# rvaser/rala

Measured on AMD Instinct MI355X. Metric: overlaps/sec (pile build + transitive reduction), higher is better.
Workload: dtype u16/u32 (+f64 compares)

## Files before the change

### rala_amd/csrc/bucket_kernels.hip

```cpp
#include <hip/hip_runtime.h>

#include <algorithm>

#include "device_utils.h"
#include "geom.h"
#include "kernels.h"
#include "scan_pass.h"

namespace rala_hip {

namespace {

constexpr uint32_t kInf = 0xFFFFFFFFu;
constexpr uint32_t kTile = 4096;
constexpr uint32_t kBlockP = 512;
constexpr uint32_t kPer = kTile / kBlockP;
constexpr uint32_t kL1Shift = 12;
constexpr uint32_t kL1Reads = 1u << kL1Shift;
constexpr uint32_t kGroupShift = 7;
constexpr uint32_t kGroupReads = 1u << kGroupShift;
constexpr uint32_t kGroupsPerPart = kL1Reads / kGroupReads;
constexpr uint32_t kKeyBits = 14;
constexpr uint32_t kCoordBits = 25;
constexpr uint32_t kCoordMax = (1u << kCoordBits) - 1u;
static_assert(kKeyBits + 2 * kCoordBits == 64, "a record is 8 bytes");

struct PartGeom {
    uint32_t shift, gpp, n_part;
};
inline PartGeom part_geom(uint32_t n_reads, const BucketTuning& bt) {
    uint32_t shift = kL1Shift;
    while (shift < kKeyBits && ((uint64_t)n_reads + (1u << shift) - 1) >> shift > 256) ++shift;
    if (bt.part_shift >= kL1Shift && bt.part_shift <= kKeyBits) shift = bt.part_shift;
    return PartGeom{shift, 1u << (shift - kGroupShift), (uint32_t)(((uint64_t)n_reads + (1u << shift) - 1) >> shift)};
}

constexpr uint32_t kCountWindow = 150u * 1024u / 4u;
inline uint32_t count_window(const BucketTuning& bt) { return bt.count_window ? bt.count_window : kCountWindow; }

__device__ __forceinline__ uint64_t pack_record(uint32_t b, uint32_t begin, uint32_t end) {
    return (uint64_t)(b & ((1u << kKeyBits) - 1u)) << (2 * kCoordBits) | (uint64_t)(begin < kCoordMax ? begin : kCoordMax) << kCoordBits |
           (uint64_t)(end < kCoordMax ? end : kCoordMax);
}
__device__ __forceinline__ uint32_t rec_key(uint64_t r) { return (uint32_t)(r >> (2 * kCoordBits)); }
__device__ __forceinline__ uint2 rec_events(uint64_t r, uint32_t shrink) {
    const uint32_t begin = (uint32_t)(r >> kCoordBits) & kCoordMax, end = (uint32_t)r & kCoordMax;
    return make_uint2((begin + shrink) << 1, ((end - shrink) << 1) | 1u);
}

__device__ __forceinline__ uint32_t segment_of(uint32_t key, bool active, uint32_t lane, uint32_t& leader) {
    const uint32_t prev = (uint32_t)__shfl_up((int)key, 1, 64);
    const bool prev_active = __shfl_up((int)active, 1, 64) != 0;
    const bool head = active && (lane == 0 || !prev_active || prev != key);
    const uint64_t heads = __ballot(head);
    const uint64_t act = __ballot(active);
    const uint64_t below = heads & ((lane == 63) ? ~0ull : ((2ull << lane) - 1ull));
    leader = below ? 63u - (uint32_t)__clzll((long long)below) : lane;
    const uint64_t after = (lane == 63) ? 0ull : ((heads | ~act) >> (lane + 1));
    const uint32_t len = after ? (uint32_t)__ffsll((unsigned long long)after) : (64u - lane);
    return head ? len : 0u;
}

constexpr uint32_t kBlockC = 1024;
constexpr uint32_t kCountPer = 8;
__global__ __launch_bounds__(kBlockC) void group_count_kernel(OvlSoA o, uint32_t n_reads, uint32_t g_lo, uint32_t n_groups, uint32_t* group_count) {
    extern __shared__ uint32_t s_hist[];
    for (uint32_t g = threadIdx.x; g < n_groups; g += kBlockC) s_hist[g] = 0;
    __syncthreads();
    constexpr uint32_t kC = kCountPer;
    const uint64_t last = o.n - 1;
    for (uint64_t i0 = (uint64_t)blockIdx.x * kBlockC * kC; i0 < o.n; i0 += (uint64_t)gridDim.x * kBlockC * kC) {
        uint32_t a[kC], b[kC];
#pragma unroll
        for (uint32_t u = 0; u < kC; ++u) {
            const uint64_t i = i0 + u * kBlockC + threadIdx.x;
            const uint64_t j = i < o.n ? i : last;
            a[u] = i < o.n ? __builtin_nontemporal_load(o.a_id + j) : kInf;
            b[u] = __builtin_nontemporal_load(o.b_id + j);
        }
#pragma unroll
        for (uint32_t u = 0; u < kC; ++u) {
            const uint32_t g = (b[u] >> kGroupShift) - g_lo;
            if (a[u] < n_reads && b[u] < n_reads && g < n_groups) atomicAdd(&s_hist[g], 1u);
        }
    }
    __syncthreads();
    for (uint32_t g = threadIdx.x; g < n_groups; g += kBlockC) {
        const uint32_t c = s_hist[g];
        if (c) atomicAdd(&group_count[g_lo + g], c);
    }
}

__device__ __forceinline__ void load4_ids(const uint32_t* p, uint64_t i0, uint64_t n, uint32_t (&out)[4]) {
    typedef uint32_t u32x4_t __attribute__((ext_vector_type(4)));
    if (i0 + 4 <= n) {
        const u32x4_t v = __builtin_nontemporal_load((const u32x4_t*)(p + i0));
        out[0] = v.x; out[1] = v.y; out[2] = v.z; out[3] = v.w;
    } else {
#pragma unroll
        for (uint32_t e = 0; e < 4; ++e) out[e] = i0 + e < n ? p[i0 + e] : kInf;
    }
}
constexpr uint32_t kCountVec = 2;
constexpr uint32_t kFlagStage = 512;
template <bool kShard>
__global__ __launch_bounds__(kBlockC) void group_count_dedupe_kernel(OvlSoA o, uint32_t n_reads, uint32_t n_groups, uint32_t* group_count,
                                                                     uint8_t* __restrict__ suspect, uint8_t* __restrict__ valid, uint32_t* list_pos,
                                                                     uint32_t* list_query, uint32_t list_cap, uint32_t* list_count,
                                                                     uint32_t world, uint32_t groups) {
    extern __shared__ uint32_t s_hist[];
    __shared__ uint32_t s_fpos[kFlagStage], s_fq[kFlagStage], s_fcnt, s_fbase;
    for (uint32_t g = threadIdx.x; g < n_groups; g += kBlockC) s_hist[g] = 0;
    if (threadIdx.x == 0) s_fcnt = 0;
    __syncthreads();
    const uint32_t lane = threadIdx.x & 63;
    auto mark = [&](uint32_t query, uint64_t at) {
        suspect[query] = 1;
        const uint32_t slot = atomicAdd(&s_fcnt, 1u);
        if (slot < kFlagStage) { s_fpos[slot] = (uint32_t)at; s_fq[slot] = query; }
    };
    constexpr uint64_t kTrip = (uint64_t)kBlockC * 4 * kCountVec;
    for (uint64_t c0 = (uint64_t)blockIdx.x * kTrip; c0 < o.n; c0 += (uint64_t)gridDim.x * kTrip) {
        uint32_t a[kCountVec][4], b[kCountVec][4];
#pragma unroll
        for (uint32_t u = 0; u < kCountVec; ++u) {
            const uint64_t i0 = c0 + ((uint64_t)u * kBlockC + threadIdx.x) * 4;
            load4_ids(o.a_id, i0, o.n, a[u]);
            load4_ids(o.b_id, i0, o.n, b[u]);
        }
#pragma unroll
        for (uint32_t u = 0; u < kCountVec; ++u) {
            const uint64_t i0 = c0 + ((uint64_t)u * kBlockC + threadIdx.x) * 4;
            uint32_t pa = (uint32_t)__shfl_up((int)a[u][3], 1, 64), pb = (uint32_t)__shfl_up((int)b[u][3], 1, 64);
            if (lane == 0 && i0 > 0 && i0 < o.n) { pa = o.a_id[i0 - 1]; pb = o.b_id[i0 - 1]; }
            bool have_prev = i0 > 0;
            uint32_t word = 0;
#pragma unroll
            for (uint32_t e = 0; e < 4; ++e) {
                const uint32_t x = a[u][e], y = b[u][e];
                const bool in = i0 + e < o.n;
                const bool ok = in && x < n_reads && y < n_reads;
                if (ok) {
                    if constexpr (kShard) {
                        atomicAdd(&s_hist[(x % world) * groups + ((x / world) >> kGroupShift)], 1u);
                        atomicAdd(&s_hist[(y % world) * groups + ((y / world) >> kGroupShift)], 1u);
                    } else {
                        if ((y >> kGroupShift) < n_groups) atomicAdd(&s_hist[y >> kGroupShift], 1u);
                    }
                }
                if (in && have_prev) {
                    const bool pok = pa < n_reads && pb < n_reads;
                    if (ok && pok) {
                        if (pa == x && y <= pb) mark(x, i0 + e);
                    } else {
                        if (x < n_reads) mark(x, i0 + e);
                        if (pa < n_reads) mark(pa, i0 + e - 1);
                    }
                }
                if (ok && x != y) word |= 1u << (8 * e);
                pa = x; pb = y; have_prev = true;
            }
            if (i0 + 4 <= o.n) *(uint32_t*)(valid + i0) = word;
            else for (uint32_t e = 0; e < 4 && i0 + e < o.n; ++e) valid[i0 + e] = (uint8_t)(word >> (8 * e));
        }
        __syncthreads();
        const uint32_t staged = s_fcnt;
        if (staged) {
            if (threadIdx.x == 0) s_fbase = staged > kFlagStage ? atomicOr(list_count, kDedupeListGivenUp) : atomicAdd(list_count, staged);
            __syncthreads();
            if (staged <= kFlagStage) {
                for (uint32_t k = threadIdx.x; k < staged; k += kBlockC) {
                    const uint32_t at = s_fbase + k;
                    if (at < list_cap) { list_pos[at] = s_fpos[k]; list_query[at] = s_fq[k]; }
                }
            }
            __syncthreads();
            if (threadIdx.x == 0) s_fcnt = 0;
            __syncthreads();
        }
    }
    for (uint32_t g = threadIdx.x; g < n_groups; g += kBlockC) {
        const uint32_t c = s_hist[g];
        if (c) atomicAdd(&group_count[g], c);
    }
}

__global__ __launch_bounds__(1024) void layout_kernel(const uint32_t* __restrict__ group_count, uint32_t n_part, uint32_t gpp,
                                                      uint32_t* __restrict__ group_base, uint32_t* __restrict__ group_cursor,
                                                      uint32_t* __restrict__ part_cursor, uint32_t* __restrict__ tile_part,
                                                      uint32_t* __restrict__ tile_lo, uint32_t* __restrict__ tile_hi, uint32_t* n_tiles) {
    __shared__ uint32_t tmp[1024 / 64 + 1];
    const uint32_t n = n_part * gpp;
    uint32_t carry = 0;
    for (uint32_t g0 = 0; g0 < n; g0 += 1024) {
        const uint32_t g = g0 + threadIdx.x;
        const uint32_t c = g < n ? group_count[g] : 0u;
        uint32_t tot;
        const uint32_t ex = block_scan_excl<1024>(c, OpAdd(), 0u, tmp, tot);
        if (g < n) {
            group_base[g] = carry + ex;
            group_cursor[g] = carry + ex;
            if (g % gpp == 0) part_cursor[g / gpp] = carry + ex;
        }
        carry += tot;
    }
    if (threadIdx.x == 0) group_base[n] = carry;
    __syncthreads();
    uint32_t tile_carry = 0;
    for (uint32_t p0 = 0; p0 < n_part; p0 += 1024) {
        const uint32_t p = p0 + threadIdx.x;
        const uint32_t lo = p < n_part ? group_base[p * gpp] : 0u;
        const uint32_t hi = p < n_part ? group_base[(p + 1u) * gpp] : 0u;
        const uint32_t tiles = (hi - lo + kTile - 1) / kTile;
        uint32_t ttot;
        const uint32_t tex = block_scan_excl<1024>(tiles, OpAdd(), 0u, tmp, ttot);
        for (uint32_t k = 0; k < tiles; ++k) {
            tile_part[tile_carry + tex + k] = p;
            tile_lo[tile_carry + tex + k] = lo + k * kTile;
            tile_hi[tile_carry + tex + k] = umin(hi, lo + (k + 1u) * kTile);
        }
        tile_carry += ttot;
    }
    if (threadIdx.x == 0) *n_tiles = tile_carry;
}

struct StageLds {
    uint64_t* stage;
    uint16_t* bin_of;
    uint32_t *hist, *off, *gbase;
    __device__ StageLds(unsigned char* base, uint32_t n_bins) {
        stage = (uint64_t*)base;
        bin_of = (uint16_t*)(stage + kTile);
        hist = (uint32_t*)(bin_of + kTile);
        off = hist + n_bins;
        gbase = off + n_bins;
    }
};
inline size_t stage_lds_bytes(uint32_t n_bins) { return (size_t)kTile * 10 + (size_t)n_bins * 12 + 16; }

__device__ __forceinline__ void stage_and_copy(StageLds& L, uint32_t n_bins, const uint64_t* rec, const uint32_t* bin, const bool* in,
                                               uint32_t* cursor, uint64_t* __restrict__ out, uint32_t* tmp) {
    for (uint32_t p = threadIdx.x; p < n_bins; p += kBlockP) L.hist[p] = 0;
    __syncthreads();
    uint32_t rank[kPer];
#pragma unroll
    for (uint32_t u = 0; u < kPer; ++u) rank[u] = in[u] ? atomicAdd(&L.hist[bin[u]], 1u) : 0u;
    __syncthreads();
    uint32_t carry = 0;
    for (uint32_t p0 = 0; p0 < n_bins; p0 += kBlockP) {
        const uint32_t p = p0 + threadIdx.x;
        const uint32_t c = p < n_bins ? L.hist[p] : 0u;
        uint32_t tot;
        const uint32_t ex = block_scan_excl<(int)kBlockP>(c, OpAdd(), 0u, tmp, tot);
        if (p < n_bins) {
            L.off[p] = carry + ex;
            L.gbase[p] = c ? atomicAdd(&cursor[p], c) : 0u;
        }
        carry += tot;
    }
    __syncthreads();
    const uint32_t total = carry;
#pragma unroll
    for (uint32_t u = 0; u < kPer; ++u) {
        if (in[u]) {
            const uint32_t at = L.off[bin[u]] + rank[u];
            L.stage[at] = rec[u];
            L.bin_of[at] = (uint16_t)bin[u];
        }
    }
    __syncthreads();
    for (uint32_t j = threadIdx.x; j < total; j += kBlockP) {
        const uint32_t p = L.bin_of[j];
        out[L.gbase[p] + (j - L.off[p])] = L.stage[j];
    }
}

__global__ __launch_bounds__(kBlockP) void l1_scatter_kernel(OvlSoA o, uint32_t n_reads, uint32_t n_part, uint32_t shift, uint32_t* part_cursor,
                                                             uint64_t* __restrict__ rec1, uint32_t* acount) {
    extern __shared__ __align__(16) unsigned char s_raw[];
    __shared__ uint32_t tmp[kBlockP / 64 + 1];
    StageLds L(s_raw, n_part);
    uint64_t rec[kPer];
    uint32_t bin[kPer];
    bool in[kPer];
    const uint32_t lane = threadIdx.x & 63;
    const uint64_t last = o.n - 1;
#pragma unroll
    for (uint32_t u = 0; u < kPer; ++u) {
        const uint64_t i = (uint64_t)blockIdx.x * kTile + u * kBlockP + threadIdx.x;
        const uint64_t j = i < o.n ? i : last;
        const uint32_t a = o.a_id[j], b = o.b_id[j];
        in[u] = i < o.n && a < n_reads && b < n_reads;
        rec[u] = pack_record(b, o.b_begin[j], o.b_end[j]);
        bin[u] = in[u] ? b >> shift : 0u;
        uint32_t leader;
        const uint32_t seg = segment_of(a, in[u], lane, leader);
        if (seg) atomicAdd(&acount[a], seg);
    }
    stage_and_copy(L, n_part, rec, bin, in, part_cursor, rec1, tmp);
}

__device__ __forceinline__ uint32_t bound_record_read(uint64_t r) { return (uint32_t)(r >> (2 * kBoundRecordCoordBits)); }

__global__ __launch_bounds__(kBlockC) void group_count_records_kernel(const uint64_t* __restrict__ records, uint64_t n, uint32_t n_reads,
                                                                      uint32_t g_lo, uint32_t n_groups, uint32_t* group_count) {
    extern __shared__ uint32_t s_hist[];
    for (uint32_t g = threadIdx.x; g < n_groups; g += kBlockC) s_hist[g] = 0;
    __syncthreads();
    constexpr uint32_t kC = kCountPer;
    for (uint64_t i0 = (uint64_t)blockIdx.x * kBlockC * kC; i0 < n; i0 += (uint64_t)gridDim.x * kBlockC * kC) {
        uint32_t key[kC];
#pragma unroll
        for (uint32_t u = 0; u < kC; ++u) {
            const uint64_t i = i0 + u * kBlockC + threadIdx.x;
            key[u] = i < n ? bound_record_read(__builtin_nontemporal_load(records + i)) : kInf;
        }
#pragma unroll
        for (uint32_t u = 0; u < kC; ++u) {
            const uint32_t g = (key[u] >> kGroupShift) - g_lo;
            if (key[u] < n_reads && g < n_groups) atomicAdd(&s_hist[g], 1u);
        }
    }
    __syncthreads();
    for (uint32_t g = threadIdx.x; g < n_groups; g += kBlockC) {
        const uint32_t c = s_hist[g];
        if (c) atomicAdd(&group_count[g_lo + g], c);
    }
}

__global__ __launch_bounds__(kBlockP) void l1_scatter_records_kernel(const uint64_t* __restrict__ records, uint64_t n, uint32_t n_reads,
                                                                     uint32_t n_part, uint32_t shift, uint32_t* part_cursor, uint64_t* __restrict__ rec1) {
    extern __shared__ __align__(16) unsigned char s_raw[];
    __shared__ uint32_t tmp[kBlockP / 64 + 1];
    StageLds L(s_raw, n_part);
    uint64_t rec[kPer];
    uint32_t bin[kPer];
    bool in[kPer];
    constexpr uint32_t kMask = (1u << kBoundRecordCoordBits) - 1u;
#pragma unroll
    for (uint32_t u = 0; u < kPer; ++u) {
        const uint64_t i = (uint64_t)blockIdx.x * kTile + u * kBlockP + threadIdx.x;
        const uint64_t r = i < n ? __builtin_nontemporal_load(records + i) : ~0ull;
        const uint32_t key = bound_record_read(r);
        in[u] = i < n && key < n_reads;
        rec[u] = pack_record(key, (uint32_t)(r >> kBoundRecordCoordBits) & kMask, (uint32_t)r & kMask);
        bin[u] = in[u] ? key >> shift : 0u;
    }
    stage_and_copy(L, n_part, rec, bin, in, part_cursor, rec1, tmp);
}

constexpr uint32_t kTileOtherBase = 0x80000000u;
__global__ __launch_bounds__(kBlockP) void l2_scatter_kernel(const uint64_t* __restrict__ rec1, const uint64_t* __restrict__ rec1b,
                                                             const uint32_t* __restrict__ tile_part,
                                                             const uint32_t* __restrict__ tile_lo, const uint32_t* __restrict__ tile_hi,
                                                             const uint32_t* __restrict__ n_tiles, uint32_t* group_cursor,
                                                             uint64_t* __restrict__ rec2, uint32_t gpp) {
    extern __shared__ __align__(16) unsigned char s_raw[];
    __shared__ uint32_t tmp[kBlockP / 64 + 1];
    if (blockIdx.x >= *n_tiles) return;
    StageLds L(s_raw, gpp);
    const uint32_t part_mask = gpp * kGroupReads - 1u;
    const uint32_t part_word = tile_part[blockIdx.x], lo = tile_lo[blockIdx.x], hi = tile_hi[blockIdx.x];
    const uint32_t part = part_word & ~kTileOtherBase;
    const uint64_t* __restrict__ src = (part_word & kTileOtherBase) ? rec1b : rec1;
    uint64_t rec[kPer];
    uint32_t bin[kPer];
    bool in[kPer];
#pragma unroll
    for (uint32_t u = 0; u < kPer; ++u) {
        const uint32_t j = lo + u * kBlockP + threadIdx.x;
        in[u] = j < hi;
        rec[u] = in[u] ? src[j] : 0ull;
        bin[u] = (rec_key(rec[u]) & part_mask) >> kGroupShift;
    }
    stage_and_copy(L, gpp, rec, bin, in, group_cursor + part * gpp, rec2, tmp);
}

__global__ __launch_bounds__(kGroupReads) void group_query_sum_kernel(const uint32_t* __restrict__ acount, uint32_t n_reads,
                                                                      uint32_t* __restrict__ qsum) {
    __shared__ uint32_t tmp[kGroupReads / 64 + 1];
    const uint32_t r = blockIdx.x * kGroupReads + threadIdx.x;
    const uint32_t v = block_reduce<(int)kGroupReads>(r < n_reads ? acount[r] : 0u, OpAdd(), 0u, tmp);
    if (threadIdx.x == 0) qsum[blockIdx.x] = v;
}

__global__ __launch_bounds__(1024) void group_event_base_kernel(const uint32_t* __restrict__ qsum, const uint32_t* __restrict__ group_base,
                                                                uint32_t n_groups, uint32_t* __restrict__ pair_base) {
    __shared__ uint32_t tmp[1024 / 64 + 1];
    uint32_t carry = 0;
    for (uint32_t g0 = 0; g0 < n_groups; g0 += 1024) {
        const uint32_t g = g0 + threadIdx.x;
        const uint32_t c = g < n_groups ? qsum[g] + (group_base[g + 1] - group_base[g]) : 0u;
        uint32_t tot;
        const uint32_t ex = block_scan_excl<1024>(c, OpAdd(), 0u, tmp, tot);
        if (g < n_groups) pair_base[g] = carry + ex;
        carry += tot;
    }
    if (threadIdx.x == 0) pair_base[n_groups] = carry;
}

__global__ __launch_bounds__(kBlockP) void final_kernel(const uint64_t* __restrict__ rec2, const uint32_t* __restrict__ group_base,
                                                        const uint32_t* __restrict__ pair_base, uint32_t n_reads,
                                                        const uint32_t* __restrict__ acount, uint32_t* __restrict__ ev_off,
                                                        uint32_t* __restrict__ ev, uint32_t shrink, uint32_t ev_shift) {
    extern __shared__ __align__(16) unsigned char s_raw[];
    __shared__ uint32_t tmp[kBlockP / 64 + 1];
    __shared__ uint32_t s_cursor[kGroupReads];
    __shared__ uint32_t s_cnt[kGroupReads];
    static_assert(kGroupReads <= kBlockP, "one thread per read of the group");
    StageLds L(s_raw, kGroupReads);
    const uint32_t g = blockIdx.x;
    if (threadIdx.x < kGroupReads) s_cnt[threadIdx.x] = 0;
    __syncthreads();
    const uint32_t lo = group_base[g], hi = group_base[g + 1];
    uint64_t first[kPer];
#pragma unroll
    for (uint32_t u = 0; u < kPer; ++u) {
        const uint32_t j = lo + u * kBlockP + threadIdx.x;
        first[u] = j < hi ? rec2[j] : 0ull;
        if (j < hi) atomicAdd(&s_cnt[rec_key(first[u]) & (kGroupReads - 1u)], 1u);
    }
    for (uint32_t j = lo + kTile + threadIdx.x; j < hi; j += kBlockP) atomicAdd(&s_cnt[rec_key(rec2[j]) & (kGroupReads - 1u)], 1u);
    __syncthreads();
    {
        const uint32_t r = g * kGroupReads + threadIdx.x;
        const bool mine = threadIdx.x < kGroupReads && r < n_reads;
        const uint32_t q = mine && acount ? acount[r] : 0u;
        const uint32_t pairs = mine ? q + s_cnt[threadIdx.x] : 0u;
        uint32_t tot;
        const uint32_t before = pair_base[g] + block_scan_excl<(int)kBlockP>(pairs, OpAdd(), 0u, tmp, tot);
        if (mine) {
            ev_off[r] = before << (1u - ev_shift);
            s_cursor[threadIdx.x] = before + q;
            if (r == n_reads - 1u) ev_off[n_reads] = (before + pairs) << (1u - ev_shift);
        }
    }
    __syncthreads();
    for (uint32_t j0 = lo; j0 < hi; j0 += kTile) {
        uint64_t pair[kPer];
        uint32_t bin[kPer];
        bool in[kPer];
#pragma unroll
        for (uint32_t u = 0; u < kPer; ++u) {
            const uint32_t j = j0 + u * kBlockP + threadIdx.x;
            in[u] = j < hi;
            const uint64_t rec = j0 == lo ? first[u] : in[u] ? rec2[j] : 0ull;
            const uint2 e = rec_events(rec, shrink);
            pair[u] = (uint64_t)e.x | (uint64_t)e.y << 32;
            bin[u] = rec_key(rec) & (kGroupReads - 1u);
        }
        stage_and_copy(L, kGroupReads, pair, bin, in, s_cursor, (uint64_t*)ev, tmp);
        __syncthreads();
    }
}

template <uint32_t kQ>
__global__ __launch_bounds__(256) void query_side_kernel(OvlSoA o, uint32_t n_reads, const uint32_t* __restrict__ ev_off,
                                                         uint32_t* written, uint32_t* __restrict__ ev, uint32_t ev_shift) {
    const uint32_t lane = threadIdx.x & 63;
    uint32_t a[kQ], b[kQ], begin[kQ], end[kQ];
#pragma unroll
    for (uint32_t u = 0; u < kQ; ++u) {
        const uint64_t i = ((uint64_t)blockIdx.x * kQ + u) * 256 + threadIdx.x;
        a[u] = kInf; b[u] = kInf; begin[u] = 0; end[u] = 0;
        if (i < o.n) { a[u] = o.a_id[i]; b[u] = o.b_id[i]; begin[u] = __builtin_nontemporal_load(o.a_begin + i); end[u] = __builtin_nontemporal_load(o.a_end + i); }
    }
    uint32_t base[kQ], leader[kQ];
    bool ok[kQ];
#pragma unroll
    for (uint32_t u = 0; u < kQ; ++u) {
        ok[u] = a[u] < n_reads && b[u] < n_reads;
        const uint32_t seg = segment_of(a[u], ok[u], lane, leader[u]);
        base[u] = 0;
        if (seg) base[u] = ev_off[a[u]] + atomicAdd(&written[a[u]], (2u >> ev_shift) * seg);
    }
#pragma unroll
    for (uint32_t u = 0; u < kQ; ++u) {
        const uint32_t at = (uint32_t)__shfl((int)base[u], (int)leader[u], 64);
        if (ok[u]) *(uint2*)(ev + ((size_t)at << ev_shift) + 2u * (lane - leader[u])) = make_uint2((begin[u] + 15u) << 1, ((end[u] - 15u) << 1) | 1u);
    }
}


__global__ __launch_bounds__(kBlockC) void shard_count_kernel(OvlSoA o, uint32_t n_reads, uint32_t world, uint32_t groups,
                                                              uint32_t n_bins, uint32_t* group_count) {
    extern __shared__ uint32_t s_hist[];
    for (uint32_t g = threadIdx.x; g < n_bins; g += kBlockC) s_hist[g] = 0;
    __syncthreads();
    constexpr uint32_t kC = kCountPer;
    const uint64_t last = o.n - 1;
    for (uint64_t i0 = (uint64_t)blockIdx.x * kBlockC * kC; i0 < o.n; i0 += (uint64_t)gridDim.x * kBlockC * kC) {
        uint32_t a[kC], b[kC];
#pragma unroll
        for (uint32_t u = 0; u < kC; ++u) {
            const uint64_t i = i0 + u * kBlockC + threadIdx.x;
            const uint64_t j = i < o.n ? i : last;
            a[u] = i < o.n ? __builtin_nontemporal_load(o.a_id + j) : kInf;
            b[u] = __builtin_nontemporal_load(o.b_id + j);
        }
#pragma unroll
        for (uint32_t u = 0; u < kC; ++u) {
            if (a[u] < n_reads && b[u] < n_reads) {
                atomicAdd(&s_hist[(a[u] % world) * groups + ((a[u] / world) >> kGroupShift)], 1u);
                atomicAdd(&s_hist[(b[u] % world) * groups + ((b[u] / world) >> kGroupShift)], 1u);
            }
        }
    }
    __syncthreads();
    for (uint32_t g = threadIdx.x; g < n_bins; g += kBlockC) {
        const uint32_t c = s_hist[g];
        if (c) atomicAdd(&group_count[g], c);
    }
}

__global__ __launch_bounds__(1024) void shard_send_layout_kernel(const uint32_t* __restrict__ group_count, ShardGeometry g,
                                                                 uint64_t* __restrict__ send, uint32_t* __restrict__ part_cursor,
                                                                 uint32_t* __restrict__ send_words) {
    __shared__ uint32_t tmp[1024 / 64 + 1];
    uint32_t block_start = 0;
    for (uint32_t p = 0; p < g.world; ++p) {
        uint32_t* header = (uint32_t*)(send + block_start);
        uint32_t carry = block_start + g.header;
        for (uint32_t g0 = 0; g0 < g.groups; g0 += 1024) {
            const uint32_t k = g0 + threadIdx.x;
            const uint32_t c = k < g.groups ? group_count[p * g.groups + k] : 0u;
            uint32_t tot;
            const uint32_t ex = block_scan_excl<1024>(c, OpAdd(), 0u, tmp, tot);
            if (k < g.groups) {
                header[k] = c;
                if (k % kGroupsPerPart == 0) part_cursor[p * g.n_part + k / kGroupsPerPart] = carry + ex;
            }
            carry += tot;
        }
        if (threadIdx.x == 0) send_words[p] = carry - block_start;
        block_start = carry;
    }
}

__global__ __launch_bounds__(kBlockP) void shard_l1_scatter_kernel(OvlSoA o, uint32_t n_reads, uint32_t world, uint32_t n_part,
                                                                   uint32_t* part_cursor, uint64_t* __restrict__ send) {
    extern __shared__ __align__(16) unsigned char s_raw[];
    __shared__ uint32_t tmp[kBlockP / 64 + 1];
    const uint32_t n_bins = world * n_part;
    StageLds L(s_raw, n_bins);
    uint64_t rec[kPer];
    uint32_t bin[kPer];
    bool in[kPer];
    const uint64_t last = o.n - 1;
    static_assert(kPer % 2 == 0, "two records per overlap");
#pragma unroll
    for (uint32_t u = 0; u < kPer / 2; ++u) {
        const uint64_t i = (uint64_t)blockIdx.x * (kTile / 2) + u * kBlockP + threadIdx.x;
        const uint64_t j = i < o.n ? i : last;
        const uint32_t a = o.a_id[j], b = o.b_id[j];
        const bool ok = i < o.n && a < n_reads && b < n_reads;
        const uint32_t la = a / world, lb = b / world;
        in[2 * u] = in[2 * u + 1] = ok;
        rec[2 * u] = pack_record(la, __builtin_nontemporal_load(o.a_begin + j), __builtin_nontemporal_load(o.a_end + j));
        rec[2 * u + 1] = pack_record(lb, __builtin_nontemporal_load(o.b_begin + j), __builtin_nontemporal_load(o.b_end + j));
        bin[2 * u] = ok ? (a - la * world) * n_part + (la >> kL1Shift) : 0u;
        bin[2 * u + 1] = ok ? (b - lb * world) * n_part + (lb >> kL1Shift) : 0u;
    }
    stage_and_copy(L, n_bins, rec, bin, in, part_cursor, send, tmp);
}

__global__ __launch_bounds__(1024) void shard_owner_layout_kernel(const uint64_t* __restrict__ base, const uint64_t* __restrict__ base_self,
                                                                  ShardBlocks blocks, ShardGeometry g,
                                                                  uint32_t* __restrict__ group_base, uint32_t* __restrict__ group_cursor,
                                                                  uint32_t* __restrict__ pair_pref, uint32_t* __restrict__ tile_part,
                                                                  uint32_t* __restrict__ tile_lo, uint32_t* __restrict__ tile_hi,
                                                                  uint32_t* n_tiles) {
    __shared__ uint32_t tmp[1024 / 64 + 1];
    auto header_of = [&](uint32_t p) { return (const uint32_t*)((p == blocks.self ? base_self : base) + blocks.off[p]); };
    uint32_t carry = 0;
    for (uint32_t g0 = 0; g0 < g.groups; g0 += 1024) {
        const uint32_t k = g0 + threadIdx.x;
        uint32_t c = 0;
        if (k < g.groups) {
            for (uint32_t p = 0; p < g.world; ++p) c += header_of(p)[k];
        }
        uint32_t tot;
        const uint32_t ex = block_scan_excl<1024>(c, OpAdd(), 0u, tmp, tot);
        if (k < g.groups) { group_base[k] = carry + ex; group_cursor[k] = carry + ex; }
        carry += tot;
    }
    if (threadIdx.x == 0) group_base[g.groups] = carry;
    const uint32_t n_pairs = g.world * g.n_part;
    uint32_t pcarry = 0;
    for (uint32_t j0 = 0; j0 < n_pairs; j0 += 1024) {
        const uint32_t j = j0 + threadIdx.x;
        uint32_t len = 0;
        if (j < n_pairs) {
            const uint32_t* header = header_of(j / g.n_part) + (j % g.n_part) * kGroupsPerPart;
            for (uint32_t k = 0; k < kGroupsPerPart; ++k) len += header[k];
        }
        uint32_t tot;
        const uint32_t ex = block_scan_excl<1024>(len, OpAdd(), 0u, tmp, tot);
        if (j < n_pairs) pair_pref[j] = pcarry + ex;
        pcarry += tot;
    }
    if (threadIdx.x == 0) pair_pref[n_pairs] = pcarry;
    __syncthreads();
    uint32_t tile_carry = 0;
    for (uint32_t j0 = 0; j0 < n_pairs; j0 += 1024) {
        const uint32_t j = j0 + threadIdx.x;
        uint32_t lo = 0, len = 0, tiles = 0;
        if (j < n_pairs) {
            const uint32_t p = j / g.n_part;
            len = pair_pref[j + 1] - pair_pref[j];
            lo = blocks.off[p] + g.header + (pair_pref[j] - pair_pref[p * g.n_part]);
            tiles = (len + kTile - 1) / kTile;
        }
        uint32_t ttot;
        const uint32_t tex = block_scan_excl<1024>(tiles, OpAdd(), 0u, tmp, ttot);
        for (uint32_t k = 0; k < tiles; ++k) {
            tile_part[tile_carry + tex + k] = (j % g.n_part) | (j / g.n_part == blocks.self ? kTileOtherBase : 0u);
            tile_lo[tile_carry + tex + k] = lo + k * kTile;
            tile_hi[tile_carry + tex + k] = umin(lo + len, lo + (k + 1u) * kTile);
        }
        tile_carry += ttot;
    }
    if (threadIdx.x == 0) *n_tiles = tile_carry;
}

}

uint32_t partition_count(uint32_t n_reads, const BucketTuning& bt) { return part_geom(n_reads, bt).n_part; }
uint32_t partition_group_slots(uint32_t n_reads, const BucketTuning& bt) { const PartGeom G = part_geom(n_reads, bt); return G.n_part * G.gpp + 2; }
size_t partition_records_needed(uint32_t, uint64_t n_overlaps) { return (size_t)n_overlaps + 64; }
size_t partition_tile_slots(uint32_t n_reads, uint64_t n_overlaps, const BucketTuning& bt) { return (size_t)(n_overlaps / kTile) + partition_count(n_reads, bt) + 4; }
bool partition_path_fits(uint32_t n_reads, uint32_t max_read_len, uint64_t n_overlaps, const BucketTuning& bt) {
    if (n_reads == 0 || n_overlaps == 0) return false;
    const PartGeom G = part_geom(n_reads, bt);
    const uint64_t n_part = G.n_part;
    return max_read_len < kCoordMax - 32u && n_part * G.gpp <= 8ull * kCountWindow &&
           stage_lds_bytes((uint32_t)n_part) <= 60u * 1024u && 2ull * n_overlaps < 0xFFFFFFF0ull && n_overlaps / n_part >= 512;
}

namespace {
struct PartitionBuffers {
    uint32_t n_part, n_groups, group_slots, shift, gpp, window;
    size_t tile_slots;
    uint32_t *group_count, *group_base, *group_cursor, *tile_part, *tile_lo, *tile_hi, *n_tiles;
    PartitionBuffers(uint32_t n_reads, uint64_t n_records, const BucketTuning& bt, uint32_t* group, uint32_t* tiles) {
        const PartGeom G = part_geom(n_reads, bt);
        n_part = G.n_part; shift = G.shift; gpp = G.gpp;
        window = std::min(n_part * gpp, count_window(bt));
        n_groups = (n_reads + kGroupReads - 1) / kGroupReads;
        group_slots = partition_group_slots(n_reads, bt);
        tile_slots = partition_tile_slots(n_reads, n_records, bt);
        group_count = group; group_base = group + group_slots; group_cursor = group + 2 * (size_t)group_slots;
        tile_part = tiles; tile_lo = tiles + tile_slots; tile_hi = tiles + 2 * tile_slots; n_tiles = tiles + 3 * tile_slots;
    }
};

hipError_t count_attribute(size_t lds_count) {
    if (lds_count + 8192 > 64 * 1024) {
        hipError_t e = hipFuncSetAttribute((const void*)group_count_kernel, hipFuncAttributeMaxDynamicSharedMemorySize, (int)lds_count);
        if (e == hipSuccess) e = hipFuncSetAttribute((const void*)group_count_dedupe_kernel<false>, hipFuncAttributeMaxDynamicSharedMemorySize, (int)lds_count);
        if (e == hipSuccess) e = hipFuncSetAttribute((const void*)group_count_records_kernel, hipFuncAttributeMaxDynamicSharedMemorySize, (int)lds_count);
        return e;
    }
    return hipSuccess;
}

void launch_partition_rest(const PartitionBuffers& B, uint32_t n_reads, const uint32_t* acount, const uint64_t* rec1, uint64_t* rec2,
                           uint32_t* ev_off, uint32_t* ev, hipStream_t s, uint32_t ev_shift, uint32_t shrink = 15u) {
    const uint32_t tiles2 = (uint32_t)(B.tile_slots - 4);
    hipLaunchKernelGGL(l2_scatter_kernel, dim3(tiles2), dim3(kBlockP), stage_lds_bytes(B.gpp), s, rec1, (const uint64_t*)nullptr,
                       (const uint32_t*)B.tile_part, (const uint32_t*)B.tile_lo, (const uint32_t*)B.tile_hi, (const uint32_t*)B.n_tiles,
                       B.group_cursor, rec2, B.gpp);
    uint32_t *qsum = B.group_count, *pair_base = B.group_cursor;
    hipLaunchKernelGGL(group_query_sum_kernel, dim3(B.n_groups), dim3(kGroupReads), 0, s, acount, n_reads, qsum);
    hipLaunchKernelGGL(group_event_base_kernel, dim3(1), dim3(1024), 0, s, (const uint32_t*)qsum, (const uint32_t*)B.group_base, B.n_groups,
                       pair_base);
    hipLaunchKernelGGL(final_kernel, dim3(B.n_groups), dim3(kBlockP), stage_lds_bytes(kGroupReads), s, (const uint64_t*)rec2,
                       (const uint32_t*)B.group_base, (const uint32_t*)pair_base, n_reads, acount, ev_off, ev, shrink, ev_shift);
}
}

bool bucket_count_can_dedupe(const OvlSoA& o, const uint8_t* valid) {
    return (((uintptr_t)o.a_id | (uintptr_t)o.b_id) & 15u) == 0 && ((uintptr_t)valid & 3u) == 0 && getenv("RALA_DEDUPE_APART") == nullptr;
}

hipError_t launch_bucket_partitioned(const OvlSoA& o, uint32_t n_reads, const BucketTuning& bt, uint32_t* acount, uint32_t* written,
                                     uint32_t* part_cursor, uint32_t* group, uint32_t* tiles, uint64_t* rec1, uint64_t* rec2,
                                     uint32_t* ev_off, uint32_t* ev, uint32_t workgroups, FillList& fills, hipStream_t s,
                                     const BucketDedupe* dedupe, uint32_t ev_shift) {
    const PartitionBuffers B(n_reads, o.n, bt, group, tiles);
    fills.add(acount, 0, (size_t)n_reads * 4);
    fills.add(written, 0, (size_t)n_reads * 4);
    fills.add(B.group_count, 0, (size_t)B.group_slots * 4);
    if (dedupe) fills.add(dedupe->suspect, 0, n_reads);
    hipError_t e = fills.launch(s);
    if (e != hipSuccess) return e;
    const uint32_t all_groups = B.n_part * B.gpp, window = B.window;
    const size_t lds_count = (size_t)window * 4;
    e = count_attribute(lds_count);
    if (e != hipSuccess) return e;
    const uint32_t chunks = (uint32_t)((o.n + kBlockC * kCountPer - 1) / (kBlockC * kCountPer));
    auto wait_for = [&](hipEvent_t ev) { return dedupe && ev ? hipStreamWaitEvent(s, ev, 0) : hipSuccess; };
    e = wait_for(dedupe ? dedupe->ids : nullptr);
    if (e != hipSuccess) return e;
    const uint32_t count_groups = (workgroups ? workgroups : 256u) * (2 * lds_count <= 150u * 1024u ? 2u : 1u);
    if (dedupe) {
        hipLaunchKernelGGL(group_count_dedupe_kernel<false>, dim3(std::min<uint32_t>(count_groups, chunks)), dim3(kBlockC), lds_count, s, o,
                           n_reads, window, B.group_count, dedupe->suspect, dedupe->valid, dedupe->list_pos,
                           dedupe->list_query, dedupe->list_cap, dedupe->list_count, 1u, 0u);
        if (dedupe->counted) {
            e = hipEventRecord(dedupe->counted, s);
            if (e != hipSuccess) return e;
        }
    } else {
        hipLaunchKernelGGL(group_count_kernel, dim3(std::min<uint32_t>(count_groups, chunks)), dim3(kBlockC), lds_count, s, o,
                           n_reads, 0u, window, B.group_count);
    }
    for (uint32_t g_lo = window; g_lo < all_groups; g_lo += window) {
        hipLaunchKernelGGL(group_count_kernel, dim3(std::min<uint32_t>(count_groups, chunks)), dim3(kBlockC), lds_count, s, o,
                           n_reads, g_lo, std::min(window, all_groups - g_lo), B.group_count);
    }
    hipLaunchKernelGGL(layout_kernel, dim3(1), dim3(1024), 0, s, (const uint32_t*)B.group_count, B.n_part, B.gpp, B.group_base, B.group_cursor,
                       part_cursor, B.tile_part, B.tile_lo, B.tile_hi, B.n_tiles);
    const uint32_t tiles1 = (uint32_t)((o.n + kTile - 1) / kTile);
    e = wait_for(dedupe ? dedupe->b_coords : nullptr);
    if (e != hipSuccess) return e;
    hipLaunchKernelGGL(l1_scatter_kernel, dim3(tiles1), dim3(kBlockP), stage_lds_bytes(B.n_part), s, o, n_reads, B.n_part, B.shift, part_cursor, rec1,
                       acount);
    launch_partition_rest(B, n_reads, acount, rec1, rec2, ev_off, ev, s, ev_shift);
    e = wait_for(dedupe ? dedupe->a_coords : nullptr);
    if (e != hipSuccess) return e;
    static const int q_per = getenv("RALA_QUERY_PER") ? atoi(getenv("RALA_QUERY_PER")) : 2;
    if (q_per == 4) hipLaunchKernelGGL(query_side_kernel<4>, dim3((uint32_t)((o.n + 1023) / 1024)), dim3(256), 0, s, o, n_reads, (const uint32_t*)ev_off, written, ev, ev_shift);
    else if (q_per == 2) hipLaunchKernelGGL(query_side_kernel<2>, dim3((uint32_t)((o.n + 511) / 512)), dim3(256), 0, s, o, n_reads, (const uint32_t*)ev_off, written, ev, ev_shift);
    else hipLaunchKernelGGL(query_side_kernel<1>, dim3((uint32_t)((o.n + 255) / 256)), dim3(256), 0, s, o, n_reads, (const uint32_t*)ev_off, written, ev, ev_shift);
    return hipGetLastError();
}

hipError_t launch_bucket_partitioned_records(const uint64_t* records, uint64_t n, uint32_t n_reads, const BucketTuning& bt, uint32_t* zero_counts,
                                             uint32_t* part_cursor, uint32_t* group, uint32_t* tiles, uint64_t* rec1, uint64_t* rec2,
                                             uint32_t* ev_off, uint32_t* ev, uint32_t workgroups, FillList& fills, hipStream_t s,
                                             uint32_t shrink, uint32_t ev_shift) {
    const PartitionBuffers B(n_reads, n, bt, group, tiles);
    fills.add(zero_counts, 0, (size_t)n_reads * 4);
    fills.add(B.group_count, 0, (size_t)B.group_slots * 4);
    hipError_t e = fills.launch(s);
    if (e != hipSuccess) return e;
    const uint32_t all_groups = B.n_part * B.gpp, window = B.window;
    const size_t lds_count = (size_t)window * 4;
    e = count_attribute(lds_count);
    if (e != hipSuccess) return e;
    const uint32_t chunks = (uint32_t)((n + kBlockC * kCountPer - 1) / (kBlockC * kCountPer));
    const uint32_t count_groups = (workgroups ? workgroups : 256u) * (2 * lds_count <= 150u * 1024u ? 2u : 1u);
    for (uint32_t g_lo = 0; g_lo < all_groups; g_lo += window) {
        hipLaunchKernelGGL(group_count_records_kernel, dim3(std::min<uint32_t>(count_groups, std::max<uint32_t>(chunks, 1u))), dim3(kBlockC),
                           lds_count, s, records, n, n_reads, g_lo, std::min(window, all_groups - g_lo), B.group_count);
    }
    hipLaunchKernelGGL(layout_kernel, dim3(1), dim3(1024), 0, s, (const uint32_t*)B.group_count, B.n_part, B.gpp, B.group_base, B.group_cursor,
                       part_cursor, B.tile_part, B.tile_lo, B.tile_hi, B.n_tiles);
    const uint32_t tiles1 = (uint32_t)((n + kTile - 1) / kTile);
    if (tiles1) {
        hipLaunchKernelGGL(l1_scatter_records_kernel, dim3(tiles1), dim3(kBlockP), stage_lds_bytes(B.n_part), s, records, n, n_reads,
                           B.n_part, B.shift, part_cursor, rec1);
    }
    launch_partition_rest(B, n_reads, zero_counts, rec1, rec2, ev_off, ev, s, ev_shift, shrink);
    return hipGetLastError();
}

bool partition_path_fits_records(uint32_t n_reads, uint32_t max_read_len, uint64_t n_records, const BucketTuning& bt) {
    return max_read_len < (1u << kBoundRecordCoordBits) - 32u && partition_path_fits(n_reads, max_read_len, (n_records + 1) / 2, bt);
}

ShardGeometry shard_geometry(uint64_t n_reads, uint32_t world) {
    ShardGeometry g;
    g.world = world;
    const uint64_t most = (n_reads + world - 1) / world;
    g.n_part = (uint32_t)std::max<uint64_t>(1, (most + kL1Reads - 1) / kL1Reads);
    g.groups = g.n_part * kGroupsPerPart;
    g.header = g.groups / 2;
    return g;
}
bool shard_path_fits(uint64_t n_reads, uint32_t max_read_len, uint32_t world) {
    if (n_reads == 0 || world == 0 || world > 64 || n_reads >= 0x7FFFFFFFull) return false;
    const ShardGeometry g = shard_geometry(n_reads, world);
    return max_read_len < kCoordMax - 32u && (uint64_t)g.world * g.groups * 4u <= 150u * 1024u &&
           stage_lds_bytes(g.world * g.n_part) <= 60u * 1024u;
}
size_t shard_send_words(const ShardGeometry& g, uint64_t n_overlaps) { return 2 * (size_t)n_overlaps + (size_t)g.world * g.header + 64; }
size_t shard_tile_slots(const ShardGeometry& g, uint64_t n_records) { return (size_t)(n_records / kTile) + (size_t)g.world * g.n_part + 4; }

hipError_t launch_shard_emit(const OvlSoA& o, uint32_t n_reads, const ShardGeometry& g, uint32_t* group_count, uint32_t* part_cursor,
                             uint64_t* send, uint32_t* send_words, uint32_t workgroups, FillList& fills, hipStream_t s,
                             const BucketDedupe* dedupe) {
    const uint32_t n_bins = g.world * g.groups;
    fills.add(group_count, 0, (size_t)n_bins * 4);
    if (dedupe) fills.add(dedupe->suspect, 0, n_reads);
    hipError_t e = fills.launch(s);
    if (e != hipSuccess) return e;
    const size_t lds_count = (size_t)n_bins * 4;
    if (lds_count + 8192 > 64 * 1024) {
        e = hipFuncSetAttribute((const void*)shard_count_kernel, hipFuncAttributeMaxDynamicSharedMemorySize, (int)lds_count);
        if (e == hipSuccess) e = hipFuncSetAttribute((const void*)group_count_dedupe_kernel<true>, hipFuncAttributeMaxDynamicSharedMemorySize, (int)lds_count);
        if (e != hipSuccess) return e;
    }
    if (o.n) {
        const uint32_t chunks = (uint32_t)((o.n + kBlockC * kCountPer - 1) / (kBlockC * kCountPer));
        const uint32_t count_groups = (workgroups ? workgroups : 256u) * (2 * lds_count <= 150u * 1024u ? 2u : 1u);
        if (dedupe) {
            hipLaunchKernelGGL(group_count_dedupe_kernel<true>, dim3(std::min<uint32_t>(count_groups, chunks)), dim3(kBlockC), lds_count, s, o,
                               n_reads, n_bins, group_count, dedupe->suspect, dedupe->valid, dedupe->list_pos, dedupe->list_query,
                               dedupe->list_cap, dedupe->list_count, g.world, g.groups);
            if (dedupe->counted) {
                e = hipEventRecord(dedupe->counted, s);
                if (e != hipSuccess) return e;
            }
        } else {
            hipLaunchKernelGGL(shard_count_kernel, dim3(std::min<uint32_t>(count_groups, chunks)), dim3(kBlockC), lds_count, s, o, n_reads,
                               g.world, g.groups, n_bins, group_count);
        }
    }
    hipLaunchKernelGGL(shard_send_layout_kernel, dim3(1), dim3(1024), 0, s, (const uint32_t*)group_count, g, send, part_cursor, send_words);
    if (o.n) {
        const uint32_t tiles1 = (uint32_t)((o.n + kTile / 2 - 1) / (kTile / 2));
        hipLaunchKernelGGL(shard_l1_scatter_kernel, dim3(tiles1), dim3(kBlockP), stage_lds_bytes(g.world * g.n_part), s, o, n_reads, g.world,
                           g.n_part, part_cursor, send);
    }
    return hipGetLastError();
}

hipError_t launch_bucket_from_blocks(const uint64_t* base, const uint64_t* base_self, const ShardBlocks& blocks, const ShardGeometry& g,
                                     uint32_t n_reads_local,
                                     uint64_t n_records, uint32_t* group, uint32_t* tiles, uint64_t* rec2, uint32_t* ev_off, uint32_t* ev,
                                     FillList& fills, hipStream_t s, uint32_t ev_shift) {
    hipError_t e = fills.launch(s);
    if (e != hipSuccess) return e;
    const uint32_t slots = g.groups + 2;
    uint32_t *group_base = group, *group_cursor = group + slots, *pair_pref = group + 2 * (size_t)slots;
    const size_t tile_slots = shard_tile_slots(g, n_records);
    uint32_t *tile_part = tiles, *tile_lo = tiles + tile_slots, *tile_hi = tiles + 2 * tile_slots, *n_tiles = tiles + 3 * tile_slots;
    hipLaunchKernelGGL(shard_owner_layout_kernel, dim3(1), dim3(1024), 0, s, base, base_self, blocks, g, group_base, group_cursor, pair_pref, tile_part,
                       tile_lo, tile_hi, n_tiles);
    hipLaunchKernelGGL(l2_scatter_kernel, dim3((uint32_t)(tile_slots - 4)), dim3(kBlockP), stage_lds_bytes(kGroupsPerPart), s, base, base_self,
                       (const uint32_t*)tile_part, (const uint32_t*)tile_lo, (const uint32_t*)tile_hi, (const uint32_t*)n_tiles, group_cursor,
                       rec2, kGroupsPerPart);
    const uint32_t n_groups = (n_reads_local + kGroupReads - 1) / kGroupReads;
    if (n_groups) {
        hipLaunchKernelGGL(final_kernel, dim3(n_groups), dim3(kBlockP), stage_lds_bytes(kGroupReads), s, (const uint64_t*)rec2,
                           (const uint32_t*)group_base, (const uint32_t*)group_base, n_reads_local, (const uint32_t*)nullptr, ev_off, ev, 15u, ev_shift);
    }
    return hipGetLastError();
}
size_t shard_group_words(const ShardGeometry& g) { return 3 * ((size_t)g.groups + 2) + (size_t)g.world * g.n_part + 2; }

}
```

Measured before the change: 7.221 billion.

## Move per-query counting into dedupe count pass and vectorize scatter/query-side loads

Computes per-query overlap counts (acount) inside the dedupe count kernel using quad-run detection across wave lanes, so the L1 scatter kernel no longer does segment reductions and atomics. When the columns are 16-byte aligned, the scatter kernel and a new query-side kernel load four overlaps per thread with vector loads. The query-side kernel reserves event slots once per run of equal query ids and writes uniform quads with wide stores. It records an 'unresolved' flag so b_id reads can be skipped when every id was valid. This adds intricate lane-run logic, which risks subtle counting and offset bugs.

```diff
diff --git a/rala_amd/csrc/bucket_kernels.hip b/rala_amd/csrc/bucket_kernels.hip
--- a/rala_amd/csrc/bucket_kernels.hip
+++ b/rala_amd/csrc/bucket_kernels.hip
@@ -1,6 +1,7 @@
 #include <hip/hip_runtime.h>
 
 #include <algorithm>
+#include <initializer_list>
 
 #include "device_utils.h"
 #include "geom.h"
@@ -61,6 +62,43 @@
     return head ? len : 0u;
 }
 
+struct QuadRuns {
+    bool uniform, joins;
+    uint32_t first_len, last_at;
+    uint32_t first_ok, last_ok;
+    uint64_t cont;
+    uint64_t w0, w1, w2;
+    __device__ __forceinline__ uint32_t joined_sum(uint64_t lanes) const {
+        return (uint32_t)__popcll(w0 & lanes) + 2u * (uint32_t)__popcll(w1 & lanes) + 4u * (uint32_t)__popcll(w2 & lanes);
+    }
+};
+__device__ __forceinline__ uint64_t lanes_up_to(uint32_t lane) { return lane >= 63u ? ~0ull : (2ull << lane) - 1ull; }
+__device__ __forceinline__ QuadRuns quad_runs(const uint32_t (&q)[4], uint32_t okm, uint32_t lane) {
+    QuadRuns r;
+    const bool e01 = q[0] == q[1], e12 = q[1] == q[2], e23 = q[2] == q[3];
+    r.uniform = e01 && e12 && e23;
+    r.first_len = !e01 ? 1u : !e12 ? 2u : !e23 ? 3u : 4u;
+    r.last_at = r.uniform ? 0u : !e23 ? 3u : !e12 ? 2u : 1u;
+    r.first_ok = (uint32_t)__popc(okm & ((1u << r.first_len) - 1u));
+    r.last_ok = (uint32_t)__popc(okm >> r.last_at);
+    const uint32_t below = (uint32_t)__shfl_up((int)q[3], 1, 64);
+    r.joins = lane > 0 && below == q[0];
+    r.cont = __ballot(r.joins && r.uniform);
+    const uint32_t w = r.joins ? r.first_ok : 0u;
+    r.w0 = __ballot((w & 1u) != 0); r.w1 = __ballot((w & 2u) != 0); r.w2 = __ballot((w & 4u) != 0);
+    return r;
+}
+__device__ __forceinline__ uint32_t quad_run_total(const QuadRuns& r, uint32_t lane) {
+    const uint64_t stop = lane >= 63u ? 0ull : (~r.cont >> (lane + 1u));
+    const uint32_t n = stop ? (uint32_t)__ffsll((unsigned long long)stop) - 1u : 63u - lane;
+    const uint32_t hi = lane + n + 1u < 64u ? lane + n + 1u : 63u;
+    return r.last_ok + r.joined_sum(lanes_up_to(hi) & ~lanes_up_to(lane));
+}
+__device__ __forceinline__ uint32_t quad_leader(const QuadRuns& r, uint32_t lane) {
+    const uint64_t heads = ~r.cont & (lanes_up_to(lane) >> 1);
+    return r.joins ? 63u - (uint32_t)__clzll((long long)heads) : lane;
+}
+
 constexpr uint32_t kBlockC = 1024;
 constexpr uint32_t kCountPer = 8;
 __global__ __launch_bounds__(kBlockC) void group_count_kernel(OvlSoA o, uint32_t n_reads, uint32_t g_lo, uint32_t n_groups, uint32_t* group_count) {
@@ -107,7 +145,7 @@
 __global__ __launch_bounds__(kBlockC) void group_count_dedupe_kernel(OvlSoA o, uint32_t n_reads, uint32_t n_groups, uint32_t* group_count,
                                                                      uint8_t* __restrict__ suspect, uint8_t* __restrict__ valid, uint32_t* list_pos,
                                                                      uint32_t* list_query, uint32_t list_cap, uint32_t* list_count,
-                                                                     uint32_t world, uint32_t groups) {
+                                                                     uint32_t world, uint32_t groups, uint32_t* acount, uint32_t* unresolved) {
     extern __shared__ uint32_t s_hist[];
     __shared__ uint32_t s_fpos[kFlagStage], s_fq[kFlagStage], s_fcnt, s_fbase;
     for (uint32_t g = threadIdx.x; g < n_groups; g += kBlockC) s_hist[g] = 0;
@@ -120,6 +158,7 @@
         if (slot < kFlagStage) { s_fpos[slot] = (uint32_t)at; s_fq[slot] = query; }
     };
     constexpr uint64_t kTrip = (uint64_t)kBlockC * 4 * kCountVec;
+    bool saw_unresolved = false;
     for (uint64_t c0 = (uint64_t)blockIdx.x * kTrip; c0 < o.n; c0 += (uint64_t)gridDim.x * kTrip) {
         uint32_t a[kCountVec][4], b[kCountVec][4];
 #pragma unroll
@@ -134,7 +173,7 @@
             uint32_t pa = (uint32_t)__shfl_up((int)a[u][3], 1, 64), pb = (uint32_t)__shfl_up((int)b[u][3], 1, 64);
             if (lane == 0 && i0 > 0 && i0 < o.n) { pa = o.a_id[i0 - 1]; pb = o.b_id[i0 - 1]; }
             bool have_prev = i0 > 0;
-            uint32_t word = 0;
+            uint32_t word = 0, okm = 0;
 #pragma unroll
             for (uint32_t e = 0; e < 4; ++e) {
                 const uint32_t x = a[u][e], y = b[u][e];
@@ -158,7 +197,20 @@
                     }
                 }
                 if (ok && x != y) word |= 1u << (8 * e);
+                if constexpr (!kShard) { okm |= (uint32_t)ok << e; saw_unresolved |= in && !ok; }
                 pa = x; pb = y; have_prev = true;
+            }
+            if constexpr (!kShard) {
+                const QuadRuns r = quad_runs(a[u], okm, lane);
+                const bool leads = !(r.joins && r.uniform);
+                const uint32_t total = leads ? quad_run_total(r, lane) : 0u;
+                if (total) atomicAdd(&acount[a[u][3]], total);
+                if (!r.uniform) {
+                    if (!r.joins && r.first_ok) atomicAdd(&acount[a[u][0]], r.first_ok);
+                    for (uint32_t e = r.first_len; e < r.last_at; ++e) {
+                        if (okm >> e & 1u) atomicAdd(&acount[a[u][e]], 1u);
+                    }
+                }
             }
             if (i0 + 4 <= o.n) *(uint32_t*)(valid + i0) = word;
             else for (uint32_t e = 0; e < 4 && i0 + e < o.n; ++e) valid[i0 + e] = (uint8_t)(word >> (8 * e));
@@ -183,6 +235,7 @@
         const uint32_t c = s_hist[g];
         if (c) atomicAdd(&group_count[g], c);
     }
+    if constexpr (!kShard) { if (saw_unresolved) *unresolved = 1u; }
 }
 
 __global__ __launch_bounds__(1024) void layout_kernel(const uint32_t* __restrict__ group_count, uint32_t n_part, uint32_t gpp,
@@ -275,6 +328,7 @@
     }
 }
 
+template <bool kVec>
 __global__ __launch_bounds__(kBlockP) void l1_scatter_kernel(OvlSoA o, uint32_t n_reads, uint32_t n_part, uint32_t shift, uint32_t* part_cursor,
                                                              uint64_t* __restrict__ rec1, uint32_t* acount) {
     extern __shared__ __align__(16) unsigned char s_raw[];
@@ -283,19 +337,44 @@
     uint64_t rec[kPer];
     uint32_t bin[kPer];
     bool in[kPer];
-    const uint32_t lane = threadIdx.x & 63;
-    const uint64_t last = o.n - 1;
-#pragma unroll
-    for (uint32_t u = 0; u < kPer; ++u) {
-        const uint64_t i = (uint64_t)blockIdx.x * kTile + u * kBlockP + threadIdx.x;
-        const uint64_t j = i < o.n ? i : last;
-        const uint32_t a = o.a_id[j], b = o.b_id[j];
-        in[u] = i < o.n && a < n_reads && b < n_reads;
-        rec[u] = pack_record(b, o.b_begin[j], o.b_end[j]);
-        bin[u] = in[u] ? b >> shift : 0u;
-        uint32_t leader;
-        const uint32_t seg = segment_of(a, in[u], lane, leader);
-        if (seg) atomicAdd(&acount[a], seg);
+    if constexpr (kVec) {
+        static_assert(kPer % 4 == 0, "groups of four overlaps");
+        uint32_t a[kPer / 4][4], b[kPer / 4][4], begin[kPer / 4][4], end[kPer / 4][4];
+#pragma unroll
+        for (uint32_t v = 0; v < kPer / 4; ++v) {
+            const uint64_t i0 = (uint64_t)blockIdx.x * kTile + ((uint64_t)v * kBlockP + threadIdx.x) * 4;
+            load4_ids(o.a_id, i0, o.n, a[v]);
+            load4_ids(o.b_id, i0, o.n, b[v]);
+            load4_ids(o.b_begin, i0, o.n, begin[v]);
+            load4_ids(o.b_end, i0, o.n, end[v]);
+        }
+#pragma unroll
+        for (uint32_t v = 0; v < kPer / 4; ++v) {
+#pragma unroll
+            for (uint32_t e = 0; e < 4; ++e) {
+                const uint32_t u = 4 * v + e;
+                in[u] = a[v][e] < n_reads && b[v][e] < n_reads;
+                rec[u] = pack_record(b[v][e], begin[v][e], end[v][e]);
+                bin[u] = in[u] ? b[v][e] >> shift : 0u;
+            }
+        }
+    } else {
+        const uint32_t lane = threadIdx.x & 63;
+        const uint64_t last = o.n - 1;
+#pragma unroll
+        for (uint32_t u = 0; u < kPer; ++u) {
+            const uint64_t i = (uint64_t)blockIdx.x * kTile + u * kBlockP + threadIdx.x;
+            const uint64_t j = i < o.n ? i : last;
+            const uint32_t a = o.a_id[j], b = o.b_id[j];
+            in[u] = i < o.n && a < n_reads && b < n_reads;
+            rec[u] = pack_record(b, o.b_begin[j], o.b_end[j]);
+            bin[u] = in[u] ? b >> shift : 0u;
+            if (acount) {
+                uint32_t leader;
+                const uint32_t seg = segment_of(a, in[u], lane, leader);
+                if (seg) atomicAdd(&acount[a], seg);
+            }
+        }
     }
     stage_and_copy(L, n_part, rec, bin, in, part_cursor, rec1, tmp);
 }
@@ -479,6 +558,63 @@
         const uint32_t at = (uint32_t)__shfl((int)base[u], (int)leader[u], 64);
         if (ok[u]) *(uint2*)(ev + ((size_t)at << ev_shift) + 2u * (lane - leader[u])) = make_uint2((begin[u] + 15u) << 1, ((end[u] - 15u) << 1) | 1u);
     }
+}
+
+typedef uint32_t pair2_t __attribute__((ext_vector_type(4), aligned(8)));
+template <bool kReadB>
+__device__ __forceinline__ void query_side_quads(const OvlSoA& o, uint32_t n_reads, const uint32_t* __restrict__ ev_off, uint32_t* written,
+                                                 uint32_t* __restrict__ ev, uint32_t ev_shift) {
+    const uint32_t lane = threadIdx.x & 63;
+    const uint64_t i0 = ((uint64_t)blockIdx.x * 256 + threadIdx.x) * 4;
+    uint32_t a[4], b[4] = {0u, 0u, 0u, 0u}, begin[4], end[4];
+    load4_ids(o.a_id, i0, o.n, a);
+    if constexpr (kReadB) load4_ids(o.b_id, i0, o.n, b);
+    load4_ids(o.a_begin, i0, o.n, begin);
+    load4_ids(o.a_end, i0, o.n, end);
+    uint32_t okm = 0;
+#pragma unroll
+    for (uint32_t e = 0; e < 4; ++e) okm |= (uint32_t)(a[e] < n_reads && b[e] < n_reads) << e;
+    const QuadRuns r = quad_runs(a, okm, lane);
+    const uint32_t unit = 2u >> ev_shift;
+    const bool leads = !(r.joins && r.uniform);
+    const uint32_t total = leads ? quad_run_total(r, lane) : 0u;
+    uint32_t last_base = 0, first_base = 0;
+    if (total) last_base = ev_off[a[3]] + atomicAdd(&written[a[3]], unit * total);
+    if (!r.uniform && !r.joins && r.first_ok) first_base = ev_off[a[0]] + atomicAdd(&written[a[0]], unit * r.first_ok);
+    const uint32_t leader = quad_leader(r, lane);
+    const uint32_t lead_base = (uint32_t)__shfl((int)last_base, (int)leader, 64);
+    const uint32_t lead_own = (uint32_t)__shfl((int)r.last_ok, (int)leader, 64);
+    if (r.joins) first_base = lead_base + unit * (lead_own + r.joined_sum((lanes_up_to(lane) >> 1) & ~lanes_up_to(leader)));
+    else if (r.uniform) first_base = last_base;
+    auto bounds = [&](uint32_t e) { return make_uint2((begin[e] + 15u) << 1, ((end[e] - 15u) << 1) | 1u); };
+    if (r.uniform && okm == 15u) {
+        uint32_t* at = ev + ((size_t)first_base << ev_shift);
+        const uint2 p0 = bounds(0), p1 = bounds(1), p2 = bounds(2), p3 = bounds(3);
+        pair2_t lo, hi;
+        lo.x = p0.x; lo.y = p0.y; lo.z = p1.x; lo.w = p1.y;
+        hi.x = p2.x; hi.y = p2.y; hi.z = p3.x; hi.w = p3.y;
+        *(pair2_t*)at = lo;
+        *(pair2_t*)(at + 4) = hi;
+        return;
+    }
+    uint32_t rank = 0;
+#pragma unroll
+    for (uint32_t e = 0; e < 4; ++e) {
+        if (e == r.last_at && !r.uniform) rank = 0;
+        if (!(okm >> e & 1u)) continue;
+        uint32_t base;
+        if (e < r.first_len) base = first_base;
+        else if (e >= r.last_at) base = last_base;
+        else { base = ev_off[a[e]] + atomicAdd(&written[a[e]], unit); rank = 0; }
+        *(uint2*)(ev + ((size_t)base << ev_shift) + 2u * rank) = bounds(e);
+        ++rank;
+    }
+}
+__global__ __launch_bounds__(256) void query_side_quads_kernel(OvlSoA o, uint32_t n_reads, const uint32_t* __restrict__ ev_off,
+                                                               uint32_t* written, uint32_t* __restrict__ ev, uint32_t ev_shift,
+                                                               const uint32_t* __restrict__ unresolved) {
+    if (unresolved == nullptr || *unresolved != 0u) query_side_quads<true>(o, n_reads, ev_off, written, ev, ev_shift);
+    else query_side_quads<false>(o, n_reads, ev_off, written, ev, ev_shift);
 }
 
 
@@ -642,6 +778,7 @@
     uint32_t n_part, n_groups, group_slots, shift, gpp, window;
     size_t tile_slots;
     uint32_t *group_count, *group_base, *group_cursor, *tile_part, *tile_lo, *tile_hi, *n_tiles;
+    uint32_t* unresolved;
     PartitionBuffers(uint32_t n_reads, uint64_t n_records, const BucketTuning& bt, uint32_t* group, uint32_t* tiles) {
         const PartGeom G = part_geom(n_reads, bt);
         n_part = G.n_part; shift = G.shift; gpp = G.gpp;
@@ -649,6 +786,7 @@
         n_groups = (n_reads + kGroupReads - 1) / kGroupReads;
         group_slots = partition_group_slots(n_reads, bt);
         tile_slots = partition_tile_slots(n_reads, n_records, bt);
+        unresolved = group + (size_t)n_part * gpp;
         group_count = group; group_base = group + group_slots; group_cursor = group + 2 * (size_t)group_slots;
         tile_part = tiles; tile_lo = tiles + tile_slots; tile_hi = tiles + 2 * tile_slots; n_tiles = tiles + 3 * tile_slots;
     }
@@ -676,6 +814,14 @@
                        pair_base);
     hipLaunchKernelGGL(final_kernel, dim3(B.n_groups), dim3(kBlockP), stage_lds_bytes(kGroupReads), s, (const uint64_t*)rec2,
                        (const uint32_t*)B.group_base, (const uint32_t*)pair_base, n_reads, acount, ev_off, ev, shrink, ev_shift);
+}
+}
+
+namespace {
+bool on_16_bytes(std::initializer_list<const void*> columns) {
+    uintptr_t bits = 0;
+    for (const void* c : columns) bits |= (uintptr_t)c;
+    return (bits & 15u) == 0;
 }
 }
 
@@ -706,7 +852,7 @@
     if (dedupe) {
         hipLaunchKernelGGL(group_count_dedupe_kernel<false>, dim3(std::min<uint32_t>(count_groups, chunks)), dim3(kBlockC), lds_count, s, o,
                            n_reads, window, B.group_count, dedupe->suspect, dedupe->valid, dedupe->list_pos,
-                           dedupe->list_query, dedupe->list_cap, dedupe->list_count, 1u, 0u);
+                           dedupe->list_query, dedupe->list_cap, dedupe->list_count, 1u, 0u, acount, B.unresolved);
         if (dedupe->counted) {
             e = hipEventRecord(dedupe->counted, s);
             if (e != hipSuccess) return e;
@@ -724,13 +870,22 @@
     const uint32_t tiles1 = (uint32_t)((o.n + kTile - 1) / kTile);
     e = wait_for(dedupe ? dedupe->b_coords : nullptr);
     if (e != hipSuccess) return e;
-    hipLaunchKernelGGL(l1_scatter_kernel, dim3(tiles1), dim3(kBlockP), stage_lds_bytes(B.n_part), s, o, n_reads, B.n_part, B.shift, part_cursor, rec1,
-                       acount);
+    const bool counted = dedupe != nullptr;
+    if (counted && on_16_bytes({o.a_id, o.b_id, o.b_begin, o.b_end})) {
+        hipLaunchKernelGGL(l1_scatter_kernel<true>, dim3(tiles1), dim3(kBlockP), stage_lds_bytes(B.n_part), s, o, n_reads, B.n_part, B.shift,
+                           part_cursor, rec1, (uint32_t*)nullptr);
+    } else {
+        hipLaunchKernelGGL(l1_scatter_kernel<false>, dim3(tiles1), dim3(kBlockP), stage_lds_bytes(B.n_part), s, o, n_reads, B.n_part, B.shift,
+                           part_cursor, rec1, counted ? (uint32_t*)nullptr : acount);
+    }
     launch_partition_rest(B, n_reads, acount, rec1, rec2, ev_off, ev, s, ev_shift);
     e = wait_for(dedupe ? dedupe->a_coords : nullptr);
     if (e != hipSuccess) return e;
     static const int q_per = getenv("RALA_QUERY_PER") ? atoi(getenv("RALA_QUERY_PER")) : 2;
-    if (q_per == 4) hipLaunchKernelGGL(query_side_kernel<4>, dim3((uint32_t)((o.n + 1023) / 1024)), dim3(256), 0, s, o, n_reads, (const uint32_t*)ev_off, written, ev, ev_shift);
+    if (on_16_bytes({o.a_id, o.b_id, o.a_begin, o.a_end})) {
+        hipLaunchKernelGGL(query_side_quads_kernel, dim3((uint32_t)((o.n + 1023) / 1024)), dim3(256), 0, s, o, n_reads, (const uint32_t*)ev_off, written,
+                           ev, ev_shift, (const uint32_t*)(counted ? B.unresolved : nullptr));
+    } else if (q_per == 4) hipLaunchKernelGGL(query_side_kernel<4>, dim3((uint32_t)((o.n + 1023) / 1024)), dim3(256), 0, s, o, n_reads, (const uint32_t*)ev_off, written, ev, ev_shift);
     else if (q_per == 2) hipLaunchKernelGGL(query_side_kernel<2>, dim3((uint32_t)((o.n + 511) / 512)), dim3(256), 0, s, o, n_reads, (const uint32_t*)ev_off, written, ev, ev_shift);
     else hipLaunchKernelGGL(query_side_kernel<1>, dim3((uint32_t)((o.n + 255) / 256)), dim3(256), 0, s, o, n_reads, (const uint32_t*)ev_off, written, ev, ev_shift);
     return hipGetLastError();
@@ -808,7 +963,7 @@
         if (dedupe) {
             hipLaunchKernelGGL(group_count_dedupe_kernel<true>, dim3(std::min<uint32_t>(count_groups, chunks)), dim3(kBlockC), lds_count, s, o,
                                n_reads, n_bins, group_count, dedupe->suspect, dedupe->valid, dedupe->list_pos, dedupe->list_query,
-                               dedupe->list_cap, dedupe->list_count, g.world, g.groups);
+                               dedupe->list_cap, dedupe->list_count, g.world, g.groups, (uint32_t*)nullptr, (uint32_t*)nullptr);
             if (dedupe->counted) {
                 e = hipEventRecord(dedupe->counted, s);
                 if (e != hipSuccess) return e;
```

Result: no change. 7.211 billion (-0.1%).
